# JNSresearcher/eddy_currents_3d

Measured on AMD Instinct MI355X. Metric: DOF*iters/s (fp64 BiCGSTAB-with-restart, 7-pt A-V operator), higher is better.
Workload: dtype f64

## Files before the change

eddy_currents_3d_amd/csrc/ec3d_context.hip:

```cpp
#include "../../include/ec3d_hip.h"
#include "ec3d_internal.hpp"
#include "ec3d_split_sweeps.hpp"
#include "ec3d_sweep_lists.hpp"

#include <climits>
#include <algorithm>
#include <array>
#include <cmath>
#include <cstdio>
#include <cstdlib>
#include <cstring>
#include <chrono>
#include <memory>
#include <mutex>
#include <optional>

static thread_local std::string g_err;
thread_local double *ec3d_itmax_print_hold = nullptr;
void ec3d_set_error(const std::string &msg) { g_err = msg; }
extern "C" const char *ec3d_last_error(void) { return g_err.c_str(); }

static int64_t round_up(int64_t v, int64_t m) { return (v + m - 1) / m * m; }

extern "C" void ec3d_format_real8(double v, char *buf) { ec3d_format_list_directed(v, buf); }
// ... 268 lines not shown
    static std::optional<int> env(const char *name)
    {
        const char *e = getenv(name);
        return e ? std::optional<int>(atoi(e)) : std::nullopt;
    }
    std::optional<int> nt = env("EC3D_NT"), keep = env("EC3D_KEEP");
    std::optional<int> xcd_map = env("EC3D_XCD_MAP"), vec_depth = env("EC3D_VEC_DEPTH");
    enum { K2, K4, K5, SPMV_PLAIN, NVEC };
    std::optional<int> nblk_k[NVEC] = {env("EC3D_NBLK_K2"), env("EC3D_NBLK_K4"), env("EC3D_NBLK_K5"), env("EC3D_NBLK_SPMV_PLAIN")};
    std::optional<int> map_k[NVEC] = {env("EC3D_MAP_K2"), env("EC3D_MAP_K4"), env("EC3D_MAP_K5"), env("EC3D_MAP_SPMV_PLAIN")};
    std::optional<int> depth_k[NVEC] = {env("EC3D_DEPTH_K2"), env("EC3D_DEPTH_K4"), env("EC3D_DEPTH_K5"),
                                        env("EC3D_DEPTH_SPMV_PLAIN")};
    std::optional<int> zmarch = env("EC3D_ZMARCH"), patch = env("EC3D_PATCH"), nblk_spmv = env("EC3D_NBLK_SPMV");
    std::optional<int> sav_patch = env("EC3D_SAV_PATCH"), sav_patch_px = env("EC3D_SAV_PATCH_PX"), sav_il = env("EC3D_SAV_IL");
    std::optional<int> fuse23 = env("EC3D_FUSE23"), fuse51 = env("EC3D_FUSE51"), k4s = env("EC3D_K4S");
};

static inline int64_t rows_streamed(const ec3d_ctx *c)
{
    return (c->A.sav && c->A.ulist) ? (c->A.ntiles_front + (int64_t)c->A.ulist_n) * EC3D_TILE : c->A.n_pad;
}

static int choose_sweep(ec3d_ctx *c)
{
    const SweepKnobs knob;
    Sweep &sw = c->sweep;
    sw = Sweep{};
    sw.bnd_last = -1;
    sw.ntiles = c->A.n_pad / EC3D_TILE;
    sw.n = c->A.n;
// ... 163 lines not shown
                c->fuse51_ok = fuse5 == 2 || (fuse5 == 1 && fuse_big);
            }
            if (use_patch) {
                ss.patch_npx = (int)(sdx / EC3D_PX);
                ss.patch_sdx = sdx;
                const int k4s = knob.k4s.value_or(1);
                const bool undivided = c->halo == 0 && !c->dist && c->nranks <= 1;
                const int64_t fuse_rows = !(k4s != 0 && A.ncls > 0) ? (int64_t)1 << 26 : undivided ? (int64_t)20 << 20 : (int64_t)1 << 25;
                const bool fuse_big = c->A.n_pad >= fuse_rows;
                const int fuse = knob.fuse23.value_or(1);
                c->fuse23_ok = fuse == 2 || (fuse == 1 && fuse_big);
                const int fuse5 = knob.fuse51.value_or(1);
                c->fuse51_ok = fuse5 == 2 || (fuse5 == 1 && fuse_big);
                c->k4s_ok = A.ncls > 0 && !A.sav && c->fuse23_ok && c->fuse51_ok && (k4s == 2 || (k4s == 1 && fuse_big));
                {
                    const int kinds = patch == 2 ? EC3D_PAIR_ALL : knob.patch ? 0 : big ? EC3D_PAIR_DEFAULT_BIG : 0;
                    const bool slab = c->halo > 0 || c->nranks > 1;
                    ss.pair = ec3d_patch_pairs_ok(tpp, ss.patch_npx, nplanes, ss.zm_pps, ss.nblk, slab, c->dist) ? kinds : 0;
                }
            }
        }
    }
    c->us_list.reset();
    c->us_host.clear();
    {
        const bool rp = ss.rp_px > 0;
        const std::vector<int32_t> &src = rp ? c->A.rp_ulist_host : c->A.ulist_host;
        if (rp) ss.ulist_n = (int)src.size();
        if (A.sav && ss.zm_tpp > 0 && ss.ulist_n > 0 && ss.nblk % 8 == 0 &&
            (int)src.size() == ss.ulist_n && (rp || ss.ulist == c->A.ulist)) {
            c->us_host = ec3d_xcd_local_order(src, ss.zm_tpp, ss.nblk);
            EC3D_HIP(upload_list(c->us_list, c->us_host));
            ss.ulist = c->us_list;
// ... 1064 lines not shown
```

eddy_currents_3d_amd/csrc/ec3d_form.hpp:

```cpp
#pragma once
#include "ec3d_internal.hpp"

enum { FMT_GENERIC = 0, FMT_DIA7 = 7, FMT_DICT7 = 107, FMT_SAV = 207 };
#define EC3D_SAV_STRIDE 16
#define EC3D_NSTAGE 4
#define EC3D_NSTAGE_RT 2

struct SpmvForm {
    int fmt;
    bool nt;
    bool zm;
    bool tail;
    bool patch;
    bool il;
    bool hs;
    bool pair;
};

inline SpmvForm ec3d_spmv_form(const MatView &A, const Sweep &sw)
{
    SpmvForm f{};
    f.fmt = A.sav ? FMT_SAV : A.nb == 7 && A.ncls > 0 ? FMT_DICT7 : A.nb == 7 ? FMT_DIA7 : FMT_GENERIC;
    f.nt = (sw.nt & 1) != 0;
    f.zm = sw.zm_tpp > 0 && sw.bnd_last < 0 && f.fmt != FMT_GENERIC;
    f.tail = f.fmt != FMT_SAV && A.has_tail;
    f.patch = f.zm && !f.tail && ((f.fmt == FMT_DICT7 && sw.patch_npx > 0) || (f.fmt == FMT_SAV && sw.rp_px > 0));
    f.il = f.zm && !f.patch && f.fmt == FMT_SAV && sw.il_planes > 0;
    f.hs = f.fmt == FMT_DICT7 && sw.halo_store != 0;
    return f;
}

inline bool ec3d_form_pair(const SpmvForm &f, const Sweep &sw, int kind)
{
    return f.patch && f.fmt == FMT_DICT7 && !f.hs && (sw.pair & kind) != 0;
}

inline size_t ec3d_form_lds(const MatView &A, const SpmvForm &f)
{
    const size_t sav_tbl = (size_t)A.ncls * EC3D_SAV_STRIDE * 8;
    if (f.il) return sav_tbl;
    if (f.patch && f.fmt == FMT_SAV) return sav_tbl + (size_t)(2 + EC3D_NSTAGE_RT) * EC3D_TILE * 8;
    if (f.patch) return (size_t)((f.fmt == FMT_DICT7 ? A.ncls * 7 + 1 : 0) & ~1) * 8 + (size_t)(f.pair ? 4 : 2) * EC3D_TILE * 8;
    if (f.fmt == FMT_DICT7) return (size_t)A.ncls * 7 * 8;
    if (f.fmt == FMT_SAV) return sav_tbl + (f.zm ? (size_t)EC3D_NSTAGE * EC3D_TILE * 8 : 0);
    return 0;
}
```

eddy_currents_3d_amd/csrc/ec3d_internal.hpp:

```cpp
#pragma once
#include <hip/hip_runtime.h>

#include "../../include/ec3d_hip.h"
#include "ec3d_own.hpp"

#include <algorithm>
#include <climits>
#include <cstdio>
#include <cstdint>
#include <string>
#include <vector>

#define EC3D_THREADS 256
#define EC3D_TILE 512
#define EC3D_SAV_MAXDOM 22
#define EC3D_MAXB 16
#define EC3D_CHUNK 64
#define EC3D_OUT_SLOTS 3
#ifndef EC3D_PX
#define EC3D_PX 128
#endif
#define EC3D_PY (EC3D_TILE / EC3D_PX)

struct MatView {
// ... 39 lines not shown
    const uint8_t *rp_flag;
    int nown;
    int64_t own_lo[4], own_hi[4];
    int64_t win_nt, win_blk, win_t0;
    int zm_pl0, zm_npl;
    int zm_plstep;
    int bnd_last;
    int halo_store;
    int part_off;
    const int32_t *ulist;
    int ulist_n;
    int il_planes = 0, il_nw = 0;
    const uint32_t *il_umask = nullptr;
    const int32_t *il_seg = nullptr;
    int pair = 0;
};

template <class SW>
__host__ __device__ inline int64_t ec3d_row_of(const SW &sw, int64_t tile, int t)
{
    if (sw.patch_npx <= 0) return tile * EC3D_TILE + 2 * (int64_t)t;
    const int64_t plane = tile / sw.zm_tpp, q = tile % sw.zm_tpp;
    const int64_t py = q / sw.patch_npx, px = q % sw.patch_npx;
    return plane * (int64_t)sw.zm_tpp * EC3D_TILE + (py * EC3D_PY + t / (EC3D_PX / 2)) * sw.patch_sdx + px * EC3D_PX +
           2 * (int64_t)(t % (EC3D_PX / 2));
}

template <class SW>
__host__ __device__ inline int64_t ec3d_phys_tile(const SW &sw, int64_t t)
{
// ... 470 lines not shown
```

eddy_currents_3d_amd/csrc/ec3d_kernels.hip:

```cpp
#include "ec3d_form.hpp"
#include "ec3d_recurrence.hpp"
#include "ec3d_sweep_lists.hpp"

#include <algorithm>
#include <cstdlib>
#include <type_traits>

typedef double d2 __attribute__((ext_vector_type(2)));
typedef double d2u __attribute__((ext_vector_type(2), aligned(8)));
typedef int i2 __attribute__((ext_vector_type(2)));

__device__ __forceinline__ double wave_sum(double v)
{
#pragma unroll
    for (int off = 32; off > 0; off >>= 1) v = v + __shfl_down(v, off, 64);
    return v;
}

template <bool PAIR> __device__ __forceinline__ int vw_tid()
{
    return PAIR ? (int)(threadIdx.x & (EC3D_THREADS - 1)) : (int)threadIdx.x;
}
template <bool PAIR> __device__ __forceinline__ int vw_half()
{
    if constexpr (PAIR) return __builtin_amdgcn_readfirstlane((int)(threadIdx.x / EC3D_THREADS));
    else return 0;
}
template <bool PAIR, class SW> __device__ __forceinline__ int vw_bid(const SW &sw)
{
    if constexpr (PAIR) return ec3d_patch_pair_virtual(sw.tpp, sw.patch_npx, (int)blockIdx.x, vw_half<PAIR>());
    else return (int)blockIdx.x;
}

template <int NV, bool PAIR = false>
__device__ __forceinline__ void block_sum(double (&v)[NV], double *lds)
{
    const int lane = threadIdx.x & 63, w = vw_tid<PAIR>() >> 6;
    if constexpr (PAIR) lds += vw_half<PAIR>() * (NV * 4);
#pragma unroll
    for (int k = 0; k < NV; ++k) {
        double t = wave_sum(v[k]);
        if (lane == 0) lds[k * 4 + w] = t;
    }
    __syncthreads();
#pragma unroll
    for (int k = 0; k < NV; ++k) v[k] = ((lds[k * 4 + 0] + lds[k * 4 + 1]) + lds[k * 4 + 2]) + lds[k * 4 + 3];
    __syncthreads();
}

template <int NV>
__device__ __forceinline__ void reduce_partials(const RedSrc &src, const int (&slot)[NV], double (&out)[NV],
                                                double *lds)
{
#pragma unroll
    for (int k = 0; k < NV; ++k) {
        double a = 0.0;
// ... 592 lines not shown
    }
#pragma unroll
    for (int m = 0; m < 5; ++m) {
        if (v0[m] != 0.0) s0 = s0 + v0[m] * xx[m].x;
        if (v1[m] != 0.0) s1 = s1 + v1[m] * xx[m].y;
    }
}

struct ZRegs {
    d2 xm, xc;
    d2 rim;
    d2 cr[2];
    double edge;
    unsigned short cc;
    uint32_t same;
};

__device__ __forceinline__ void stage_issue(const double *gp, double *stg, int k)
{
    __builtin_amdgcn_global_load_lds((const __attribute__((address_space(1))) void *)gp,
                                     (__attribute__((address_space(3))) void *)(stg + k * EC3D_TILE +
                                                                                (threadIdx.x >> 6) * 128),
                                     16, 0, 0);
}
__device__ __forceinline__ d2 stage_read(const double *stg, int k)
{
    return *reinterpret_cast<const d2 *>(stg + k * EC3D_TILE + 2 * threadIdx.x);
}
#define EC3D_VM_DRAIN                                                                                                  \
    do {                                                                                                               \
// ... 688 lines not shown
    }
    const d2 s = patch_sums<FMT>(c, tbl, cc, zm, ym, left, cx, right, yp, zp);
    s0 = s.x;
    s1 = s.y;
    *reinterpret_cast<d2 *>(nxt + 2 * t) = zp;
    z.xm = cx;
    z.xc = zp;
    if constexpr (RQ == PP_RIM_CARRIED) {
        if (rimrow) rimn_r = x.rpair(r + kdz + roff);
        V::to_carry(rimn_r, z.cr);
    } else {
        z.rim = x.form(rimn_r);
        z.edge = x.form(en_r);
    }
}
template <int FMT, bool NTB, bool PAIR, class V>
__device__ __forceinline__ void patch_pair(const MatDev<FMT> &A, const double *tbl, double *pbuf, int step, const V &x,
                                           int64_t r, int64_t tile, bool first, ZRegs &z, double &s0, double &s1,
                                           d2 &ctr)
{
    if constexpr (PatchReq<V>::mode == PP_BRANCHY) patch_pair_branchy<FMT, NTB, PAIR>(A, tbl, pbuf, step, x, r, tile, first, z, s0, s1, ctr);
    else patch_pair_fused<FMT, NTB, PAIR>(A, tbl, pbuf, step, x, r, tile, first, z, s0, s1, ctr);
}

template <int FMT, bool ZM, bool TAIL, bool NTB, bool PATCH, bool PAIR = false, class V, class SW>
__device__ __forceinline__ void spmv_pair(const MatDev<FMT> &A, const SW &sw, const PatchPos &pp, const double *tbl,
                                          double *stg, int &step, const V &x, int64_t r, int64_t tile, bool first,
                                          ZRegs &z, double &s0, double &s1, d2 &ctr)
{
    if constexpr (FMT == FMT_SAV && ZM && PATCH) {
// ... 441 lines not shown
        EC3D_IDLE2(s0, s1);
        acc[0] = acc[0] + q0 * q0;
        acc[0] = acc[0] + q1 * q1;
        acc[1] = acc[1] + s0 * q.x;
        acc[1] = acc[1] + s1 * q.y;
        acc[2] = acc[2] + s0 * s0;
        acc[2] = acc[2] + s1 * s1;
    });
    block_sum<3, PAIR>(acc, lds);
    {
        const int pslot_[3] = {P_SS, P_D2, P_D3};
        publish_partials<3, PAIR>(sw, part, pslot_, acc, lds);
    }
}

template <int FMT, bool NT, bool ZM, bool TAIL, bool PATCH, bool HS = false, bool PAIR = false>
__global__ __launch_bounds__(EC3D_WG_THREADS) __attribute__((amdgpu_waves_per_eu(4))) void k51_p_spmv_dot(
    MatDev<FMT> A, EC3D_SWEEP_OF(ZM) sw, RedSrc src, SolverState *st, int it, const double *__restrict__ rv,
    const double *__restrict__ p_old, const double *__restrict__ ap_old, double *__restrict__ p_new,
    double *__restrict__ ap_new, double *__restrict__ r0, double *__restrict__ part, double *hist, int64_t hist_cap)
{
    __shared__ double lds[(PAIR ? 2 : 1) * 8];
    EC3D_TBL_DECL;
    const int slot[2] = {P_RR, P_RR0N};
    PartialsEarly<2> pe;
    partials_request<2, PAIR>(src, slot, pe);
    const double bnorm = st->bnorm, tol = st->tol, alpha = st->alpha, omega = st->omega, rr0 = st->rr0[it & 1];
    TableEarly te;
    table_request<FMT>(A, te);
    {
        int si, kind;
// ... 13 lines not shown
    }
    const Ec3dBeta bs = ec3d_beta_step(alpha, omega, d[1], rr0, d[0], bnorm, tol);
    const double beta = bs.beta;
    const bool restart = bs.restart;
    if (lead) st->rr0[(it + 1) & 1] = bs.rr0_next;
    if (lead && restart) st->restarts = st->restarts + 1;
    table_store<FMT>(A, te, tbl);
    ZRegs zr;
    PatchPos pp{};
    int pstep = 0;
    double acc[1] = {0.0};
    walk_spmv<FMT, ZM, FMT != FMT_SAV, PATCH, PAIR>(A, sw, pp, [&](int64_t tile, auto fc) {
        EC3D_ROW_S;
        double s0, s1;
        d2 pc;
        spmv_pair<FMT, ZM, TAIL, NT, PATCH, PAIR>(A, sw, pp, tbl, stg, pstep, VecFusedP{rv, p_old, ap_old, beta, omega, restart}, r, tile,
                                            (bool)fc, zr, s0, s1, pc);
        d2 q = restart ? pc : load2<NT>(r0 + r);
        store2<NT>(p_new, r, nst, pc.x, pc.y);
        if (restart) store2<NT>(r0, r, nst, pc.x, pc.y);
        if constexpr (HS && FMT == FMT_DICT7 && ZM && PATCH) {
            if (sw.hs_mask) {
                const int64_t pl = tile / sw.tpp, kdz = A.off[6];
                const VecFusedP xp{rv, p_old, ap_old, beta, omega, restart};
                if ((sw.hs_mask & 1) && pl == 0) *reinterpret_cast<d2 *>(p_new + r - kdz) = xp.pair(r - kdz);
                if ((sw.hs_mask & 2) && pl == sw.hs_last) *reinterpret_cast<d2 *>(p_new + r + kdz) = xp.pair(r + kdz);
            }
        }
        store2<NT>(ap_new, r, nst, s0, s1);
        EC3D_MASK2(r, sw, s0, s1);
        EC3D_IDLE2(s0, s1);
        acc[0] = acc[0] + s0 * q.x;
        acc[0] = acc[0] + s1 * q.y;
    });
    block_sum<1, PAIR>(acc, lds);
    {
        const int pslot_[1] = {P_D1};
        publish_partials<1, PAIR>(sw, part, pslot_, acc, lds);
    }
}

template <bool NT>
__global__ __launch_bounds__(EC3D_THREADS) void k4_x_r_update(SweepV sw, RedSrc src_ss, RedSrc src, SolverState *st,
                                                              int it, const double *__restrict__ p,
                                                              const double *__restrict__ sv,
                                                              const double *__restrict__ as,
                                                              const double *__restrict__ r0, double *__restrict__ x,
                                                              double *__restrict__ rv, double *__restrict__ part,
                                                              double *hist, int64_t hist_cap)
{
// ... 446 lines not shown
    z.rp_sdy = sw.rp_sdy;
    z.rp_flag = sw.rp_flag;
    z.il_planes = sw.il_planes;
    z.il_nw = sw.il_nw;
    z.il_umask = sw.il_umask;
    z.il_seg = sw.il_seg;
    return z;
}
static constexpr bool form_possible(const SpmvForm &f)
{
    const bool table = f.fmt == FMT_DICT7 || f.fmt == FMT_SAV;
    return (!f.tail || f.fmt != FMT_SAV) && (!f.zm || f.fmt != FMT_GENERIC) && (!f.patch || (f.zm && !f.tail && table)) &&
           (!f.il || (f.zm && !f.patch && f.fmt == FMT_SAV)) && (!f.hs || f.fmt == FMT_DICT7);
}
struct SpmvFamily {
    static constexpr bool hs = false;
    static constexpr int pair_kind = EC3D_PAIR_K13;
    static constexpr bool has(const SpmvForm &f) { return form_possible(f) && !f.hs; }
};
struct FusedFamily {
    static constexpr bool hs = true;
    static constexpr bool has(const SpmvForm &f) { return form_possible(f) && f.zm && f.patch && !f.tail; }
};
struct Fused23Family : FusedFamily { static constexpr int pair_kind = EC3D_PAIR_K23; };
struct Fused51Family : FusedFamily { static constexpr int pair_kind = EC3D_PAIR_K51; };
struct K4sFamily {
    static constexpr bool hs = false;
    static constexpr int pair_kind = EC3D_PAIR_K4S;
    static constexpr bool has(const SpmvForm &f) { return FusedFamily::has(f) && f.fmt == FMT_DICT7 && !f.hs; }
};
template <int FMT_, bool NT_, bool ZM_, bool TAIL_, bool PATCH_, bool HS_, bool PAIR_> struct FormTag {
    static constexpr int FMT = FMT_;
    static constexpr bool NT = NT_, ZM = ZM_, TAIL = TAIL_, PATCH = PATCH_, HS = HS_, PAIR = PAIR_;
    static constexpr int threads = PAIR_ ? 2 * EC3D_THREADS : EC3D_THREADS;
    static int grid(const Sweep &sw) { return PAIR_ ? sw.nblk / 2 : sw.nblk; }
};
template <class FAMILY, class LAUNCH>
static void launch_form(const char *kernel, const MatView &A, const Sweep &sw, LAUNCH &&launch, int pair_kind = FAMILY::pair_kind)
{
    SpmvForm f = ec3d_spmv_form(A, sw);
    f.hs = f.hs && FAMILY::hs;
    f.pair = ec3d_form_pair(f, sw, pair_kind);
    const size_t lds = ec3d_form_lds(A, f);
    bool found = false;
    auto with_fmt = [&](auto FMT) {
        tag_bools([&](auto NT, auto ZM, auto TAIL, auto PATCH, auto IL, auto HS, auto PAIR) {
            constexpr SpmvForm cf{decltype(FMT)::value,   decltype(NT)::value, decltype(ZM)::value, decltype(TAIL)::value,
                                  decltype(PATCH)::value, decltype(IL)::value, decltype(HS)::value, decltype(PAIR)::value};
            if constexpr (FAMILY::has(cf) && (!cf.pair || (cf.patch && cf.fmt == FMT_DICT7 && !cf.hs))) {
                using T = FormTag<cf.fmt, cf.nt, cf.zm, cf.tail || cf.il, cf.patch, cf.hs, cf.pair>;
                found = true;
                if constexpr (cf.zm) launch(T{}, mat_dev<cf.fmt>(A), sweep_z(sw), lds);
                else launch(T{}, mat_dev<cf.fmt>(A), sw, lds);
            }
        }, f.nt, f.zm, f.tail, f.patch, f.il, f.hs, f.pair);
    };
    switch (f.fmt) {
    case FMT_SAV: with_fmt(std::integral_constant<int, FMT_SAV>{}); break;
    case FMT_DICT7: with_fmt(std::integral_constant<int, FMT_DICT7>{}); break;
    case FMT_DIA7: with_fmt(std::integral_constant<int, FMT_DIA7>{}); break;
    default: with_fmt(std::integral_constant<int, FMT_GENERIC>{});
    }
    if (!found) {
        char msg[160];
        snprintf(msg, sizeof msg, "%s: no kernel instance for the form fmt=%d nt=%d zm=%d tail=%d patch=%d il=%d hs=%d", kernel,
                 f.fmt, f.nt, f.zm, f.tail, f.patch, f.il, f.hs);
        ec3d_set_error(msg);
    }
}
static inline SweepV sweep_v(const Sweep &sw)
// ... 90 lines not shown
                     const double *ap, double *sv, double *as, double *part, hipStream_t s)
{
    launch_form<Fused23Family>("k23_s_spmv_dots", A, sw, [&](auto t, const auto &Ad, const auto &swk, size_t lds) {
        using T = decltype(t);
        k23_s_spmv_dots<T::FMT, T::NT, T::ZM, T::TAIL, T::PATCH, T::HS, T::PAIR><<<T::grid(sw), T::threads, lds, s>>>(
            Ad, swk, src, st, it, r, ap, sv, as, part);
    });
}

void ec3d_launch_k51(const MatView &A, const Sweep &sw, const RedSrc &src, SolverState *st, int it, const double *r,
                     const double *p_old, const double *ap_old, double *p_new, double *ap_new, double *r0, double *part,
                     double *hist, int64_t hist_cap, hipStream_t s)
{
    launch_form<Fused51Family>("k51_p_spmv_dot", A, sw, [&](auto t, const auto &Ad, const auto &swk, size_t lds) {
        using T = decltype(t);
        k51_p_spmv_dot<T::FMT, T::NT, T::ZM, T::TAIL, T::PATCH, T::HS, T::PAIR><<<T::grid(sw), T::threads, lds, s>>>(
            Ad, swk, src, st, it, r, p_old, ap_old, p_new, ap_new, r0, part, hist, hist_cap);
    });
}

void ec3d_launch_k4(const Sweep &sw, const RedSrc &src_ss, const RedSrc &src, SolverState *st, int it,
                    const double *p, const double *sv, const double *as, const double *r0, double *x, double *r,
                    double *part, double *hist, int64_t hist_cap, hipStream_t s)
{
    tag_bools([&](auto NT) {
        k4_x_r_update<decltype(NT)::value><<<sw.nblk, EC3D_THREADS, 0, s>>>(sweep_v(sw), src_ss, src, st, it, p, sv, as, r0, x, r, part,
                                                                          hist, hist_cap);
    }, nt_of(sw));
}

void ec3d_launch_k4d(const Sweep &sw, const RedSrc &src_ss, const RedSrc &src, SolverState *st, int it, int ne, int xm,
// ... 121 lines not shown
```

eddy_currents_3d_amd/csrc/ec3d_measure.hip:

```cpp
#include "../../include/ec3d_hip.h"
#include "ec3d_internal.hpp"

#include <algorithm>
#include <climits>
#include <cmath>
#include <cstdio>
#include <cstdlib>
#include <cstring>
#include <mutex>
#include <string>

extern "C" int ec3d_time_iterations(ec3d_handle c, int32_t iters, double *ms_total)
{
    int rc = ec3d_need_matrix(c, "ec3d_time_iterations");
    if (rc) return rc;
    if ((rc = ec3d_single_rank_only(c, "ec3d_time_iterations"))) return rc;
    const MatView A = c->A.view();
    c->hist_cap = 0;
    if ((rc = ec3d_launch_begin(c, A, -1.0))) return rc;
    EC3D_HIP(hipEventRecord(c->t0, c->stream));
    (void)ec3d_run_open(c, 1, iters);
    for (int it = 1; it <= iters; ++it) ec3d_launch_iteration(c, A, it);
    EC3D_HIP(hipEventRecord(c->t1, c->stream));
    EC3D_HIP(hipGetLastError());
// ... 18 lines not shown
    int rc = ec3d_need_matrix(c, "ec3d_get_fusion");
    if (rc) return rc;
    if (k2_in_k3) *k2_in_k3 = ec3d_fused23(c) ? 1 : 0;
    if (k5_in_k1) *k5_in_k1 = ec3d_fused51(c) ? 1 : 0;
    return 0;
}

extern "C" int ec3d_get_patch_rows(ec3d_handle c, int kind, int32_t *rows)
{
    int rc = ec3d_need_matrix(c, "ec3d_get_patch_rows");
    if (rc) return rc;
    if (kind < 0 || kind > 4 || !rows) return 2;
    const Sweep &ss = c->sweep_s;
    const bool dict = c->A.ncls > 0 && !c->A.sav;
    *rows = !(ss.patch_npx > 0 && dict) ? 0 : (ss.pair & (1 << kind)) ? 2 * EC3D_PY : EC3D_PY;
    return 0;
}

extern "C" int ec3d_get_x_interval(ec3d_handle c, int32_t *iterations)
{
    int rc = ec3d_need_matrix(c, "ec3d_get_x_interval");
    if (rc) return rc;
    if (iterations) *iterations = ec3d_xdefer(c);
    return 0;
}

extern "C" int ec3d_get_x_groups(ec3d_handle c, int32_t *second_stream, int32_t *groups_launched)
{
    int rc = ec3d_need_matrix(c, "ec3d_get_x_groups");
    if (rc) return rc;
// ... 115 lines not shown
```

eddy_currents_3d_amd/csrc/ec3d_sweep_lists.hpp:

```cpp
#pragma once
#include <algorithm>
#include <array>
#include <cmath>
#include <cstdint>
#include <cstdlib>
#include <vector>

inline double ec3d_pick_patch_shape(int64_t sdx, int64_t sdy, int64_t tile, int &px_out, int &py_out)
{
    double best = 0.0;
    px_out = py_out = 0;
    if (sdx % 2) return 0.0;
    for (int64_t px = 4; px <= std::min<int64_t>(sdx, 256); px += 2) {
        if (sdx % px) continue;
        if (px < 32 && px != sdx) continue;
        const int64_t py = tile / px;
        if (py < 2) continue;
        const int64_t npy = (sdy + py - 1) / py;
        const double eff = (double)(px * py) / tile * (double)sdy / (double)(npy * py);
        const bool better = eff > best + 1e-9 ||
                            (eff > best - 1e-9 && std::llabs(px - 128) < std::llabs((int64_t)px_out - 128));
        if (better) {
            best = std::max(best, eff);
            px_out = (int)px;
// ... 69 lines not shown
    if (cpx % (2 * npx)) return false;
    if (nblk % tpp) return false;
    const int64_t nseg = nblk / tpp;
    return nseg * pps == nplanes;
}
EC3D_PAIR_HD inline int ec3d_patch_pair_virtual(int tpp, int npx, int phys, int half)
{
    const int cpx = tpp >> 3, hc = cpx >> 1;
    const int c = phys & 7, sgp = phys >> 3;
    const int seg = sgp / hc, jj = sgp - seg * hc;
    const int pr = jj / npx, px = jj - pr * npx;
    return 8 * (seg * cpx + (2 * pr + half) * npx + px) + c;
}
enum { EC3D_PAIR_SPMV = 1, EC3D_PAIR_K23 = 2, EC3D_PAIR_K51 = 4, EC3D_PAIR_K4S = 8, EC3D_PAIR_K13 = 16, EC3D_PAIR_ALL = 31 };
enum { EC3D_PAIR_DEFAULT_BIG = EC3D_PAIR_SPMV | EC3D_PAIR_K23 };

inline int64_t ec3d_zm_segments(int64_t want_s, int64_t cols, int64_t max_seg, bool explicit_request)
{
    int64_t nseg = 1;
    if (explicit_request) {
        nseg = std::max<int64_t>(1, (want_s + cols / 2) / cols);
    } else {
        const int64_t fit = want_s / cols;
        nseg = (fit >= 1 && 6 * cols * fit >= 5 * want_s) ? fit : (3 * want_s + 2 * cols - 1) / (2 * cols);
    }
    return std::min<int64_t>(nseg, max_seg);
}

inline uint32_t ec3d_il_bit(const uint32_t *um, int nw, int64_t col, int64_t k)
{
// ... 103 lines not shown
```

eddy_currents_3d_amd/solver.py:

```python
from __future__ import annotations

import ctypes as C
import os

import numpy as np

PKG = os.path.dirname(os.path.abspath(__file__))
LIBPATH = os.environ.get("EC3D_LIB") or os.path.join(PKG, "libec3d_hip.so")


class EC3DError(RuntimeError):
    pass


class Geom(C.Structure):
    _fields_ = [("n_pad", C.c_int32), ("tile", C.c_int32), ("nblk", C.c_int32),
                ("threads", C.c_int32), ("xcd_group", C.c_int32), ("zm_tpp", C.c_int32),
                ("zm_pps", C.c_int32), ("ntiles_front", C.c_int32), ("ulist_n", C.c_int32),
                ("patch_x", C.c_int32), ("patch_y", C.c_int32), ("patch_sdx", C.c_int32),
                ("patch_pitch", C.c_int32), ("patch_sdy", C.c_int32)]


class MatrixInfo(C.Structure):
    _fields_ = [("n", C.c_int64), ("n_pad", C.c_int64), ("nnz", C.c_int64), ("nbands", C.c_int32),
# ... 40 lines not shown
           "ec3d_iterate_begin", "ec3d_iterate", "ec3d_get_fusion", "ec3d_get_x_interval", "ec3d_get_x_groups", "ec3d_get_k4_form", "ec3d_get_band_placement", "ec3d_get_vector_placement", "ec3d_place_vectors", "ec3d_set_format", "ec3d_set_stream",
           "ec3d_assemble_poisson_slab", "ec3d_vector_layout", "ec3d_adopt_vectors",
           "ec3d_dist_configure", "ec3d_dist_step", "ec3d_dist_set_boundary_rows", "ec3d_read_state_async", "ec3d_read_state", "ec3d_get_restart_count", "ec3d_set_zmarch", "ec3d_can_overlap",
           "ec3d_rhs_step", "ec3d_post_update", "ec3d_assemble_slab", "ec3d_vtk_fields", "ec3d_vtk_fields_begin", "ec3d_vtk_fields_wait",
           "ec3d_set_structured", "ec3d_get_row_map", "ec3d_get_ulist", "ec3d_probe_csr",
           "ec3d_device_synchronize", "ec3d_format_real8",
           "ec3d_multi_create", "ec3d_multi_destroy", "ec3d_multi_ranks", "ec3d_multi_slab", "ec3d_multi_set_format",
           "ec3d_multi_assemble_poisson", "ec3d_multi_assemble", "ec3d_multi_set_matrix_csr", "ec3d_multi_size",
           "ec3d_multi_upload", "ec3d_multi_download", "ec3d_multi_solve", "ec3d_multi_solve_resident",
           "ec3d_multi_rhs_step", "ec3d_multi_post_update", "ec3d_multi_vtk_fields", "ec3d_multi_vtk_fields_begin",
           "ec3d_multi_vtk_fields_wait", "ec3d_multi_iterate_begin",
           "ec3d_multi_iterate", "ec3d_multi_synchronize", "ec3d_true_residual", "ec3d_multi_true_residual", "ec3d_get_visit_order", "ec3d_probe_csr_multi", "ec3d_multi_spmv", "ec3d_multi_api_calls", "ec3d_multi_plan", "ec3d_multi_halo_rows", "ec3d_rccl_unique_id", "ec3d_multi_create_rank", "ec3d_format_real8_gfortran", "ec3d_multi_iterate_timed", "ec3d_multi_rccl_info",
           "ec3d_set_preconditioner", "ec3d_get_preconditioner", "ec3d_precond_apply", "ec3d_set_u_rhs",
           "ec3d_set_precond_precision", "ec3d_get_precond_precision", "ec3d_set_precond_coarsening",
           "ec3d_get_precond_coarsening", "ec3d_set_precond_grid", "ec3d_get_precond_grid",
           "ec3d_domain_integrals", "ec3d_field_energy", "ec3d_domain_linkage", "ec3d_get_class_runs", "ec3d_get_patch_rows", "ec3d_set_guess_history", "ec3d_get_guess_history"]
U_RHS = {"reference": 0, "all": 1}
PRECOND = {"none": 0, "mg": 1, "block-mg": 2}
PRECOND_E_MATRIX, PRECOND_E_COARSE = 20, 21
PRECOND_PRECISION = {"fp64": 0, "fp32": 1}
PRECOND_COARSENING = {"rediscretize": 0, "aggregate": 1}

_f64 = np.ctypeslib.ndpointer(np.float64, flags="C_CONTIGUOUS")
_i32 = np.ctypeslib.ndpointer(np.int32, flags="C_CONTIGUOUS")
_i8 = np.ctypeslib.ndpointer(np.int8, flags="C_CONTIGUOUS")
_lib = None


def torch_hip_runtime():
    import importlib.util
    try:
# ... 99 lines not shown
    L.ec3d_get_k4_form.argtypes = [hp, C.POINTER(C.c_int32)]
    L.ec3d_get_band_placement.argtypes = [hp, C.c_int32, hp, C.POINTER(C.c_int32), C.POINTER(C.c_int32)]
    L.ec3d_get_vector_placement.argtypes = [hp, C.c_int32, hp, C.POINTER(C.c_int32), C.POINTER(C.c_int32), C.POINTER(C.c_double)]
    L.ec3d_place_vectors.argtypes = [hp, C.c_int32]
    L.ec3d_set_format.argtypes = [hp, C.c_int]
    L.ec3d_set_structured.argtypes = [hp, C.c_int]
    L.ec3d_get_row_map.argtypes = [hp, _i32]
    L.ec3d_dist_set_boundary_rows.argtypes = [hp, C.c_int32, np.ctypeslib.ndpointer(np.int64, flags="C_CONTIGUOUS"),
                                              np.ctypeslib.ndpointer(np.int64, flags="C_CONTIGUOUS"),
                                              C.POINTER(C.c_int32)]
    L.ec3d_probe_csr.argtypes = [C.c_int32, _f64, _i32, _i32, C.POINTER(CsrProbe)]
    L.ec3d_probe_csr_multi.argtypes = [C.c_int32, _f64, _i32, _i32, C.c_int32, C.POINTER(C.c_int32)]
    L.ec3d_get_ulist.argtypes = [hp, _i32]
    L.ec3d_get_class_runs.argtypes = [hp, C.POINTER(C.c_int64), hp, C.c_int64]
    L.ec3d_get_patch_rows.argtypes = [hp, C.c_int, C.POINTER(C.c_int32)]
    L.ec3d_set_stream.argtypes = [hp, hp]
    L.ec3d_assemble_poisson_slab.argtypes = [hp, C.c_int32, C.c_int32, C.c_int32, C.c_int32, C.c_int32, _f64, _f64]
    L.ec3d_vector_layout.argtypes = [hp] + [C.POINTER(C.c_int64)] * 4
    L.ec3d_adopt_vectors.argtypes = [hp, hp]
    L.ec3d_dist_configure.argtypes = [hp, C.c_int32, hp, hp]
    L.ec3d_dist_step.argtypes = [hp, C.c_int32, C.c_int32, C.c_double]
    L.ec3d_read_state_async.argtypes = [hp, C.c_void_p]
    L.ec3d_read_state.argtypes = [hp, C.POINTER(C.c_int32), C.POINTER(C.c_int32), C.POINTER(C.c_double)]
    L.ec3d_get_restart_count.argtypes = [hp, C.POINTER(C.c_int32)]
    L.ec3d_get_visit_order.argtypes = [hp, C.c_int, C.POINTER(C.c_int32), C.POINTER(C.c_int64), hp, hp]
    L.ec3d_true_residual.argtypes = [hp, C.POINTER(C.c_double), C.POINTER(C.c_double)]
    L.ec3d_multi_true_residual.argtypes = [hp, C.POINTER(C.c_double), C.POINTER(C.c_double)]
    L.ec3d_multi_create.argtypes = [C.POINTER(hp), C.c_int32, hp]
    L.ec3d_multi_destroy.argtypes = [hp]
    L.ec3d_multi_ranks.argtypes = [hp]
# ... 201 lines not shown
        return off, tiles[:tot.value]

    def class_runs(self) -> np.ndarray:
        cnt = C.c_int64(0)
        _chk(self.L, self.L.ec3d_get_class_runs(self.h, C.byref(cnt), None, 0), "ec3d_get_class_runs")
        out = np.zeros(cnt.value, np.uint8)
        if cnt.value:
            _chk(self.L, self.L.ec3d_get_class_runs(self.h, C.byref(cnt), out.ctypes.data, out.size), "ec3d_get_class_runs")
        return out

    def patch_rows(self, kind: int = 0) -> int:
        rows = C.c_int32(0)
        _chk(self.L, self.L.ec3d_get_patch_rows(self.h, int(kind), C.byref(rows)), "ec3d_get_patch_rows")
        return rows.value

    def set_zmarch(self, on: bool):
        _chk(self.L, self.L.ec3d_set_zmarch(self.h, int(bool(on))), "ec3d_set_zmarch")

    def set_workgroups(self, nblk: int):
        _chk(self.L, self.L.ec3d_set_workgroups(self.h, int(nblk)), "ec3d_set_workgroups")

    def solve(self, b, x0, tolerance, itmax, hist_cap: int = 0):
        x = np.array(x0, dtype=np.float64, copy=True)
        it = C.c_int32(0)
        hist = np.full((max(hist_cap, 1), 2), np.nan)
        _chk(self.L, self.L.ec3d_solve(self.h, np.ascontiguousarray(b, np.float64), x, float(tolerance),
                                       int(itmax), C.byref(it), hist.ctypes.data if hist_cap else None,
                                       hist_cap), "ec3d_solve")
        return x, it.value, hist[:hist_cap]

# ... 525 lines not shown
```

include/ec3d_hip.h:

```cpp
#ifndef EC3D_HIP_H
#define EC3D_HIP_H
#include <stdint.h>
#ifdef __cplusplus
extern "C" {
#endif

void sprsbcgstabwr_(double *valA, int32_t *irow, int32_t *jcol, int32_t *n, double *b, double *x,
                    double *tolerance, int32_t *itmax, int32_t *iter);
void ec3d_invalidate(void);

typedef struct ec3d_ctx *ec3d_handle;

int ec3d_create(ec3d_handle *h, int device);
int ec3d_destroy(ec3d_handle h);
const char *ec3d_last_error(void);

int ec3d_set_matrix_csr(ec3d_handle h, int32_t n, const double *valA, const int32_t *irow,
                        const int32_t *jcol);

int ec3d_assemble(ec3d_handle h, int32_t sdx, int32_t sdy, int32_t sdz, const int8_t *geoPHYS,
                  const int32_t *geoPHYS_C, const double *valPHYS, int32_t nsub_glob,
                  const double *BND, const double *delta, double dt);

int ec3d_assemble_poisson(ec3d_handle h, int32_t sdx, int32_t sdy, int32_t sdz, const double *BND,
// ... 167 lines not shown
    int32_t threads;
    int32_t xcd_group;
    int32_t zm_tpp;
    int32_t zm_pps;
    int32_t ntiles_front;
    int32_t ulist_n;
    int32_t patch_x, patch_y;
    int32_t patch_sdx;
    int32_t patch_pitch;
    int32_t patch_sdy;
} ec3d_geom;
int ec3d_get_reduction_geometry(ec3d_handle h, int which, ec3d_geom *g);
int ec3d_get_ulist(ec3d_handle h, int32_t *tiles);
int ec3d_get_class_runs(ec3d_handle h, int64_t *count, uint8_t *flags, int64_t cap);
int ec3d_get_patch_rows(ec3d_handle h, int kind, int32_t *rows);
int ec3d_get_visit_order(ec3d_handle h, int which, int32_t *nwg, int64_t *total, int32_t *offsets, int32_t *tiles);
int ec3d_set_zmarch(ec3d_handle h, int on);
int ec3d_set_workgroups(ec3d_handle h, int32_t nblk);

typedef struct {
    int64_t n, n_pad, nnz;
    int32_t nbands;
    int32_t band_offset[16];
    int64_t tail_rows, tail_entries_padded;
    int64_t device_bytes;
    int32_t dict_classes;
} ec3d_matrix_info;
int ec3d_get_matrix_info(ec3d_handle h, ec3d_matrix_info *info);

int ec3d_get_band_placement(ec3d_handle h, int32_t cap, double *candidate_us, int32_t *tried, int32_t *kept);
// ... 45 lines not shown
```

Measured before the change: 50.76 billion.

## Recompute A·p_old on the fly in fused k51 kernel instead of loading it

Adds a patch_pair_apc path to the fused k51 p-update/SpMV/dot kernel. It recomputes the A·p_old product for the next plane from a second LDS-staged buffer of p_old, rather than streaming the stored ap_old vector from global memory. The path is enabled by default on large undivided dictionary-format problems, and pairing is also turned on for k51 there. A ds_bpermute-based wave reduction is added for the block sum. The trade is extra LDS use and stencil arithmetic in exchange for less global memory traffic in a bandwidth-bound fp64 kernel.

```diff
diff --git a/eddy_currents_3d_amd/csrc/ec3d_context.hip b/eddy_currents_3d_amd/csrc/ec3d_context.hip
--- a/eddy_currents_3d_amd/csrc/ec3d_context.hip
+++ b/eddy_currents_3d_amd/csrc/ec3d_context.hip
@@ -306,6 +306,7 @@
     std::optional<int> zmarch = env("EC3D_ZMARCH"), patch = env("EC3D_PATCH"), nblk_spmv = env("EC3D_NBLK_SPMV");
     std::optional<int> sav_patch = env("EC3D_SAV_PATCH"), sav_patch_px = env("EC3D_SAV_PATCH_PX"), sav_il = env("EC3D_SAV_IL");
     std::optional<int> fuse23 = env("EC3D_FUSE23"), fuse51 = env("EC3D_FUSE51"), k4s = env("EC3D_K4S");
+    std::optional<int> k51_ap = env("EC3D_K51_AP");
 };
 
 static inline int64_t rows_streamed(const ec3d_ctx *c)
@@ -499,9 +500,15 @@
                 c->fuse51_ok = fuse5 == 2 || (fuse5 == 1 && fuse_big);
                 c->k4s_ok = A.ncls > 0 && !A.sav && c->fuse23_ok && c->fuse51_ok && (k4s == 2 || (k4s == 1 && fuse_big));
                 {
-                    const int kinds = patch == 2 ? EC3D_PAIR_ALL : knob.patch ? 0 : big ? EC3D_PAIR_DEFAULT_BIG : 0;
-                    const bool slab = c->halo > 0 || c->nranks > 1;
-                    ss.pair = ec3d_patch_pairs_ok(tpp, ss.patch_npx, nplanes, ss.zm_pps, ss.nblk, slab, c->dist) ? kinds : 0;
+                    const bool inst = undivided && A.ncls > 0 && !A.sav;
+                    ss.k51_ap = inst && knob.k51_ap.value_or(big && EC3D_K51_AP_DEFAULT_BIG) != 0 ? 1 : 0;
+                }
+                const bool slab = c->halo > 0 || c->nranks > 1;
+                const bool pairs_ok = ec3d_patch_pairs_ok(tpp, ss.patch_npx, nplanes, ss.zm_pps, ss.nblk, slab, c->dist);
+                if (!knob.k51_ap && !(pairs_ok && !(knob.patch && patch != 2))) ss.k51_ap = 0;
+                {
+                    const int kinds = patch == 2 ? EC3D_PAIR_ALL : knob.patch ? 0 : !big ? 0 : EC3D_PAIR_DEFAULT_BIG | (ss.k51_ap ? EC3D_PAIR_K51 : 0);
+                    ss.pair = pairs_ok ? kinds : 0;
                 }
             }
         }
diff --git a/eddy_currents_3d_amd/csrc/ec3d_form.hpp b/eddy_currents_3d_amd/csrc/ec3d_form.hpp
--- a/eddy_currents_3d_amd/csrc/ec3d_form.hpp
+++ b/eddy_currents_3d_amd/csrc/ec3d_form.hpp
@@ -1,5 +1,6 @@
 #pragma once
 #include "ec3d_internal.hpp"
+#include "ec3d_sweep_lists.hpp"
 
 enum { FMT_GENERIC = 0, FMT_DIA7 = 7, FMT_DICT7 = 107, FMT_SAV = 207 };
 #define EC3D_SAV_STRIDE 16
@@ -15,6 +16,7 @@
     bool il;
     bool hs;
     bool pair;
+    bool apc;
 };
 
 inline SpmvForm ec3d_spmv_form(const MatView &A, const Sweep &sw)
@@ -35,12 +37,29 @@
     return f.patch && f.fmt == FMT_DICT7 && !f.hs && (sw.pair & kind) != 0;
 }
 
+inline bool ec3d_form_apc(const SpmvForm &f, const Sweep &sw)
+{
+    return f.patch && f.fmt == FMT_DICT7 && !f.hs && sw.k51_ap != 0;
+}
+
+inline SpmvForm ec3d_family_form(const MatView &A, const Sweep &sw, bool fam_hs, int pair_kind, bool fam_apc)
+{
+    SpmvForm f = ec3d_spmv_form(A, sw);
+    f.hs = f.hs && fam_hs;
+    f.pair = ec3d_form_pair(f, sw, pair_kind);
+    f.apc = fam_apc && ec3d_form_apc(f, sw);
+    return f;
+}
+inline SpmvForm ec3d_k51_form(const MatView &A, const Sweep &sw) { return ec3d_family_form(A, sw, true, EC3D_PAIR_K51, true); }
+
 inline size_t ec3d_form_lds(const MatView &A, const SpmvForm &f)
 {
     const size_t sav_tbl = (size_t)A.ncls * EC3D_SAV_STRIDE * 8;
     if (f.il) return sav_tbl;
     if (f.patch && f.fmt == FMT_SAV) return sav_tbl + (size_t)(2 + EC3D_NSTAGE_RT) * EC3D_TILE * 8;
-    if (f.patch) return (size_t)((f.fmt == FMT_DICT7 ? A.ncls * 7 + 1 : 0) & ~1) * 8 + (size_t)(f.pair ? 4 : 2) * EC3D_TILE * 8;
+    if (f.patch)
+        return (size_t)((f.fmt == FMT_DICT7 ? A.ncls * 7 + 1 : 0) & ~1) * 8 +
+               (f.apc ? (size_t)4 * ((f.pair ? 2 : 1) * EC3D_PY + 2) * EC3D_PX * 8 : (size_t)(f.pair ? 4 : 2) * EC3D_TILE * 8);
     if (f.fmt == FMT_DICT7) return (size_t)A.ncls * 7 * 8;
     if (f.fmt == FMT_SAV) return sav_tbl + (f.zm ? (size_t)EC3D_NSTAGE * EC3D_TILE * 8 : 0);
     return 0;
diff --git a/eddy_currents_3d_amd/csrc/ec3d_internal.hpp b/eddy_currents_3d_amd/csrc/ec3d_internal.hpp
--- a/eddy_currents_3d_amd/csrc/ec3d_internal.hpp
+++ b/eddy_currents_3d_amd/csrc/ec3d_internal.hpp
@@ -77,6 +77,7 @@
     const uint32_t *il_umask = nullptr;
     const int32_t *il_seg = nullptr;
     int pair = 0;
+    int k51_ap = 0;
 };
 
 template <class SW>
diff --git a/eddy_currents_3d_amd/csrc/ec3d_kernels.hip b/eddy_currents_3d_amd/csrc/ec3d_kernels.hip
--- a/eddy_currents_3d_amd/csrc/ec3d_kernels.hip
+++ b/eddy_currents_3d_amd/csrc/ec3d_kernels.hip
@@ -16,6 +16,18 @@
     for (int off = 32; off > 0; off >>= 1) v = v + __shfl_down(v, off, 64);
     return v;
 }
+__device__ __forceinline__ double wave_sum_fresh(double v)
+{
+    int lane;
+    asm volatile("v_mbcnt_lo_u32_b32 %0, -1, 0\n\tv_mbcnt_hi_u32_b32 %0, -1, %0" : "=v"(lane));
+#pragma unroll
+    for (int off = 32; off > 0; off >>= 1) {
+        const int src = (lane + off < 64 ? lane + off : lane) << 2;
+        const int lo = __builtin_amdgcn_ds_bpermute(src, __double2loint(v)), hi = __builtin_amdgcn_ds_bpermute(src, __double2hiint(v));
+        v = v + __hiloint2double(hi, lo);
+    }
+    return v;
+}
 
 template <bool PAIR> __device__ __forceinline__ int vw_tid()
 {
@@ -32,14 +44,14 @@
     else return (int)blockIdx.x;
 }
 
-template <int NV, bool PAIR = false>
+template <int NV, bool PAIR = false, bool FRESH = false>
 __device__ __forceinline__ void block_sum(double (&v)[NV], double *lds)
 {
     const int lane = threadIdx.x & 63, w = vw_tid<PAIR>() >> 6;
     if constexpr (PAIR) lds += vw_half<PAIR>() * (NV * 4);
 #pragma unroll
     for (int k = 0; k < NV; ++k) {
-        double t = wave_sum(v[k]);
+        double t = FRESH ? wave_sum_fresh(v[k]) : wave_sum(v[k]);
         if (lane == 0) lds[k * 4 + w] = t;
     }
     __syncthreads();
@@ -662,6 +674,8 @@
     double edge;
     unsigned short cc;
     uint32_t same;
+    d2 pc;
+    double pedge;
 };
 
 __device__ __forceinline__ void stage_issue(const double *gp, double *stg, int k)
@@ -1380,6 +1394,127 @@
         z.edge = x.form(en_r);
     }
 }
+template <int FMT, bool PAIR>
+__device__ __forceinline__ void patch_pair_apc(const MatDev<FMT> &A, const double *tbl, double *pbuf, int step, const VecFusedP &x,
+                                               int64_t r, int64_t tile, bool first, bool up, ZRegs &z, double &s0, double &s1,
+                                               d2 &ctr)
+{
+    static_assert(FMT == FMT_DICT7, "patch_pair_apc: the dictionary form only");
+    typedef VecFusedP V;
+    constexpr int PY = PAIR ? 2 * EC3D_PY : EC3D_PY, BUF = (PY + 2) * EC3D_PX;
+    const int t = threadIdx.x, y = t / EC3D_HX, q = t % EC3D_HX;
+    double *cur = pbuf + (step & 1) * BUF + EC3D_PX, *nxt = pbuf + ((step + 1) & 1) * BUF + EC3D_PX;
+    double *pcur = cur + 2 * BUF, *pnxt = nxt + 2 * BUF;
+    const int trim = y == 0 ? t - EC3D_HX : t + EC3D_HX;
+    const int64_t sdx = A.off[5], kdz = A.off[6], tpp = kdz / EC3D_TILE;
+    const bool calc = up && !x.restart;
+    const double *__restrict__ pup = x.p + kdz;
+    unsigned short cc, cn = 0;
+    {
+        const bool kept = !first && ((z.same >> (8 * (unsigned)((tile + tpp) & 3))) & 0xFFu) != 0;
+        uint32_t w = 0;
+        if (A.same && up) w = ((const __attribute__((address_space(4))) uint32_t *)(uintptr_t)A.same)[(tile + 2 * tpp) >> 2];
+        if (first) cc = *reinterpret_cast<const unsigned short *>(A.cls + r);
+        else cc = z.cc;
+        if (up) {
+            if (kept) cn = cc;
+            else cn = *reinterpret_cast<const unsigned short *>(A.cls + r + kdz);
+        }
+        z.same = w;
+    }
+    V::Raw2 zp_r{};
+    if (first) zp_r = x.rpair(r + kdz);
+    else zp_r.q = *reinterpret_cast<const d2u *>(x.rv + r + kdz);
+    d2 p2 = d2{0.0, 0.0};
+    if (!first && calc) p2 = *reinterpret_cast<const d2u *>(pup + r + kdz);
+    const bool edge = q == 0 || q == EC3D_HX - 1;
+    const int64_t eoff = q == 0 ? -1 : 2;
+    V::Raw1 e_r{};
+    if (edge && first) e_r = x.rat(r + eoff);
+    const bool rimrow = y == 0 || y == PY - 1;
+    const int64_t roff = y == 0 ? -sdx : sdx;
+    V::Raw2 rimc_r{};
+    if (rimrow && first) rimc_r = x.rpair(r + roff);
+    d2 zm, cx;
+    if (first) {
+        const V::Raw2 zm_r = x.rpair(r - kdz), cx_r = x.rpair(r);
+        zm = x.form(zm_r);
+        cx = x.form(cx_r);
+        *reinterpret_cast<d2 *>(cur + 2 * t) = cx;
+        const d2 rimc = x.form(rimc_r);
+        if (rimrow) *reinterpret_cast<d2 *>(cur + 2 * trim) = rimc;
+    } else {
+        cx = z.xc;
+    }
+    EC3D_PATCH_BARRIER;
+    if (!first) zm = *reinterpret_cast<const d2 *>(nxt + 2 * t);
+    const d2 ym = *reinterpret_cast<const d2 *>(cur + 2 * (t - EC3D_HX));
+    const d2 yp = *reinterpret_cast<const d2 *>(cur + 2 * (t + EC3D_HX));
+    ctr = cx;
+    double left, right;
+    {
+        const double ev = first ? x.form(e_r) : z.edge;
+        const double l = __shfl_up(cx.y, 1, 64), rr = __shfl_down(cx.x, 1, 64);
+        left = q != 0 ? l : ev;
+        right = q != EC3D_HX - 1 ? rr : ev;
+    }
+    d2 prim = d2{0.0, 0.0};
+    if (!first) {
+        const d2 pym = *reinterpret_cast<const d2 *>(pcur + 2 * (t - EC3D_HX));
+        const d2 pyp = *reinterpret_cast<const d2 *>(pcur + 2 * (t + EC3D_HX));
+        const double pl = __shfl_up(z.pc.y, 1, 64), pr = __shfl_down(z.pc.x, 1, 64);
+        const double pleft = q != 0 ? pl : z.pedge, pright = q != EC3D_HX - 1 ? pr : z.pedge;
+        const d2 pm = *reinterpret_cast<const d2 *>(pnxt + 2 * t);
+        const d2 a = patch_sums<FMT>(nullptr, tbl, cn, pm, pym, pleft, z.pc, pright, pyp, p2);
+        zp_r.pv = z.pc;
+        zp_r.a = d2{calc ? a.x : 0.0, calc ? a.y : 0.0};
+        prim = y == 0 ? pym : pyp;
+    }
+    const d2 zp = x.form(zp_r);
+    V::Raw2 rimn_r{};
+    V::Raw1 en_r{};
+    d2 prim2 = d2{0.0, 0.0};
+    double pe2 = 0.0;
+    if (first && calc) p2 = *reinterpret_cast<const d2u *>(pup + r + kdz);
+    if (rimrow) {
+        if (first) {
+            rimn_r = x.rpair(r + kdz + roff);
+        } else {
+            rimn_r.q = *reinterpret_cast<const d2u *>(x.rv + r + kdz + roff);
+            if (!x.restart) rimn_r.a = *reinterpret_cast<const d2u *>(x.ap + r + kdz + roff);
+        }
+        if (calc) prim2 = *reinterpret_cast<const d2u *>(pup + r + kdz + roff);
+    }
+    if (edge) {
+        if (first) {
+            en_r = x.rat(r + kdz + eoff);
+        } else {
+            en_r.q = x.rv[r + kdz + eoff];
+            if (!x.restart) en_r.a = x.ap[r + kdz + eoff];
+        }
+        if (calc) pe2 = pup[r + kdz + eoff];
+    }
+    if (!first) {
+        rimn_r.pv = prim;
+        en_r.pv = z.pedge;
+    }
+    const d2 s = patch_sums<FMT>(nullptr, tbl, cc, zm, ym, left, cx, right, yp, zp);
+    s0 = s.x;
+    s1 = s.y;
+    *reinterpret_cast<d2 *>(nxt + 2 * t) = zp;
+    *reinterpret_cast<d2 *>(pnxt + 2 * t) = p2;
+    if (first) *reinterpret_cast<d2 *>(pcur + 2 * t) = zp_r.pv;
+    z.xc = zp;
+    z.pc = p2;
+    z.cc = cn;
+    z.edge = x.form(en_r);
+    z.pedge = pe2;
+    const d2 rimn = x.form(rimn_r);
+    if (rimrow) {
+        *reinterpret_cast<d2 *>(nxt + 2 * trim) = rimn;
+        *reinterpret_cast<d2 *>(pnxt + 2 * trim) = prim2;
+    }
+}
 template <int FMT, bool NTB, bool PAIR, class V>
 __device__ __forceinline__ void patch_pair(const MatDev<FMT> &A, const double *tbl, double *pbuf, int step, const V &x,
                                            int64_t r, int64_t tile, bool first, ZRegs &z, double &s0, double &s1,
@@ -1851,7 +1986,7 @@
     }
 }
 
-template <int FMT, bool NT, bool ZM, bool TAIL, bool PATCH, bool HS = false, bool PAIR = false>
+template <int FMT, bool NT, bool ZM, bool TAIL, bool PATCH, bool HS = false, bool PAIR = false, bool APC = false>
 __global__ __launch_bounds__(EC3D_WG_THREADS) __attribute__((amdgpu_waves_per_eu(4))) void k51_p_spmv_dot(
     MatDev<FMT> A, EC3D_SWEEP_OF(ZM) sw, RedSrc src, SolverState *st, int it, const double *__restrict__ rv,
     const double *__restrict__ p_old, const double *__restrict__ ap_old, double *__restrict__ p_new,
@@ -1895,8 +2030,12 @@
         EC3D_ROW_S;
         double s0, s1;
         d2 pc;
-        spmv_pair<FMT, ZM, TAIL, NT, PATCH, PAIR>(A, sw, pp, tbl, stg, pstep, VecFusedP{rv, p_old, ap_old, beta, omega, restart}, r, tile,
-                                            (bool)fc, zr, s0, s1, pc);
+        if constexpr (APC)
+            patch_pair_apc<FMT, PAIR>(A, tbl, stg, pstep++, VecFusedP{rv, p_old, ap_old, beta, omega, restart}, r, tile, (bool)fc,
+                                      tile + sw.tpp < sw.ntiles, zr, s0, s1, pc);
+        else
+            spmv_pair<FMT, ZM, TAIL, NT, PATCH, PAIR>(A, sw, pp, tbl, stg, pstep, VecFusedP{rv, p_old, ap_old, beta, omega, restart}, r, tile,
+                                                (bool)fc, zr, s0, s1, pc);
         d2 q = restart ? pc : load2<NT>(r0 + r);
         store2<NT>(p_new, r, nst, pc.x, pc.y);
         if (restart) store2<NT>(r0, r, nst, pc.x, pc.y);
@@ -1914,7 +2053,7 @@
         acc[0] = acc[0] + s0 * q.x;
         acc[0] = acc[0] + s1 * q.y;
     });
-    block_sum<1, PAIR>(acc, lds);
+    block_sum<1, PAIR, APC>(acc, lds);
     {
         const int pslot_[1] = {P_D1};
         publish_partials<1, PAIR>(sw, part, pslot_, acc, lds);
@@ -2391,46 +2530,50 @@
            (!f.il || (f.zm && !f.patch && f.fmt == FMT_SAV)) && (!f.hs || f.fmt == FMT_DICT7);
 }
 struct SpmvFamily {
-    static constexpr bool hs = false;
+    static constexpr bool hs = false, apc = false;
     static constexpr int pair_kind = EC3D_PAIR_K13;
     static constexpr bool has(const SpmvForm &f) { return form_possible(f) && !f.hs; }
 };
 struct FusedFamily {
-    static constexpr bool hs = true;
+    static constexpr bool hs = true, apc = false;
     static constexpr bool has(const SpmvForm &f) { return form_possible(f) && f.zm && f.patch && !f.tail; }
 };
 struct Fused23Family : FusedFamily { static constexpr int pair_kind = EC3D_PAIR_K23; };
-struct Fused51Family : FusedFamily { static constexpr int pair_kind = EC3D_PAIR_K51; };
+struct Fused51Family : FusedFamily {
+    static constexpr int pair_kind = EC3D_PAIR_K51;
+    static constexpr bool apc = true;
+};
+static_assert(Fused51Family::hs && Fused51Family::apc && Fused51Family::pair_kind == EC3D_PAIR_K51, "ec3d_k51_form (ec3d_form.hpp)");
 struct K4sFamily {
-    static constexpr bool hs = false;
+    static constexpr bool hs = false, apc = false;
     static constexpr int pair_kind = EC3D_PAIR_K4S;
     static constexpr bool has(const SpmvForm &f) { return FusedFamily::has(f) && f.fmt == FMT_DICT7 && !f.hs; }
 };
-template <int FMT_, bool NT_, bool ZM_, bool TAIL_, bool PATCH_, bool HS_, bool PAIR_> struct FormTag {
+template <int FMT_, bool NT_, bool ZM_, bool TAIL_, bool PATCH_, bool HS_, bool PAIR_, bool APC_> struct FormTag {
     static constexpr int FMT = FMT_;
-    static constexpr bool NT = NT_, ZM = ZM_, TAIL = TAIL_, PATCH = PATCH_, HS = HS_, PAIR = PAIR_;
+    static constexpr bool NT = NT_, ZM = ZM_, TAIL = TAIL_, PATCH = PATCH_, HS = HS_, PAIR = PAIR_, APC = APC_;
     static constexpr int threads = PAIR_ ? 2 * EC3D_THREADS : EC3D_THREADS;
     static int grid(const Sweep &sw) { return PAIR_ ? sw.nblk / 2 : sw.nblk; }
 };
 template <class FAMILY, class LAUNCH>
 static void launch_form(const char *kernel, const MatView &A, const Sweep &sw, LAUNCH &&launch, int pair_kind = FAMILY::pair_kind)
 {
-    SpmvForm f = ec3d_spmv_form(A, sw);
-    f.hs = f.hs && FAMILY::hs;
-    f.pair = ec3d_form_pair(f, sw, pair_kind);
+    const SpmvForm f = ec3d_family_form(A, sw, FAMILY::hs, pair_kind, FAMILY::apc);
     const size_t lds = ec3d_form_lds(A, f);
     bool found = false;
     auto with_fmt = [&](auto FMT) {
-        tag_bools([&](auto NT, auto ZM, auto TAIL, auto PATCH, auto IL, auto HS, auto PAIR) {
-            constexpr SpmvForm cf{decltype(FMT)::value,   decltype(NT)::value, decltype(ZM)::value, decltype(TAIL)::value,
-                                  decltype(PATCH)::value, decltype(IL)::value, decltype(HS)::value, decltype(PAIR)::value};
-            if constexpr (FAMILY::has(cf) && (!cf.pair || (cf.patch && cf.fmt == FMT_DICT7 && !cf.hs))) {
-                using T = FormTag<cf.fmt, cf.nt, cf.zm, cf.tail || cf.il, cf.patch, cf.hs, cf.pair>;
+        tag_bools([&](auto NT, auto ZM, auto TAIL, auto PATCH, auto IL, auto HS, auto PAIR, auto APC) {
+            constexpr SpmvForm cf{decltype(FMT)::value,   decltype(NT)::value, decltype(ZM)::value,   decltype(TAIL)::value,
+                                  decltype(PATCH)::value, decltype(IL)::value, decltype(HS)::value,   decltype(PAIR)::value,
+                                  decltype(APC)::value};
+            constexpr bool cube2d = cf.patch && cf.fmt == FMT_DICT7 && !cf.hs;
+            if constexpr (FAMILY::has(cf) && (!cf.pair || cube2d) && (!cf.apc || (cube2d && FAMILY::apc))) {
+                using T = FormTag<cf.fmt, cf.nt, cf.zm, cf.tail || cf.il, cf.patch, cf.hs, cf.pair, cf.apc>;
                 found = true;
                 if constexpr (cf.zm) launch(T{}, mat_dev<cf.fmt>(A), sweep_z(sw), lds);
                 else launch(T{}, mat_dev<cf.fmt>(A), sw, lds);
             }
-        }, f.nt, f.zm, f.tail, f.patch, f.il, f.hs, f.pair);
+        }, f.nt, f.zm, f.tail, f.patch, f.il, f.hs, f.pair, f.apc);
     };
     switch (f.fmt) {
     case FMT_SAV: with_fmt(std::integral_constant<int, FMT_SAV>{}); break;
@@ -2551,7 +2694,7 @@
 {
     launch_form<Fused51Family>("k51_p_spmv_dot", A, sw, [&](auto t, const auto &Ad, const auto &swk, size_t lds) {
         using T = decltype(t);
-        k51_p_spmv_dot<T::FMT, T::NT, T::ZM, T::TAIL, T::PATCH, T::HS, T::PAIR><<<T::grid(sw), T::threads, lds, s>>>(
+        k51_p_spmv_dot<T::FMT, T::NT, T::ZM, T::TAIL, T::PATCH, T::HS, T::PAIR, T::APC><<<T::grid(sw), T::threads, lds, s>>>(
             Ad, swk, src, st, it, r, p_old, ap_old, p_new, ap_new, r0, part, hist, hist_cap);
     });
 }
diff --git a/eddy_currents_3d_amd/csrc/ec3d_measure.hip b/eddy_currents_3d_amd/csrc/ec3d_measure.hip
--- a/eddy_currents_3d_amd/csrc/ec3d_measure.hip
+++ b/eddy_currents_3d_amd/csrc/ec3d_measure.hip
@@ -1,5 +1,6 @@
 #include "../../include/ec3d_hip.h"
 #include "ec3d_internal.hpp"
+#include "ec3d_form.hpp"
 
 #include <algorithm>
 #include <climits>
@@ -56,6 +57,15 @@
     const Sweep &ss = c->sweep_s;
     const bool dict = c->A.ncls > 0 && !c->A.sav;
     *rows = !(ss.patch_npx > 0 && dict) ? 0 : (ss.pair & (1 << kind)) ? 2 * EC3D_PY : EC3D_PY;
+    return 0;
+}
+
+extern "C" int ec3d_get_k51_ap_form(ec3d_handle c, int32_t *computed)
+{
+    int rc = ec3d_need_matrix(c, "ec3d_get_k51_ap_form");
+    if (rc) return rc;
+    if (!computed) return 2;
+    *computed = ec3d_fused51(c) && ec3d_k51_form(c->A.view(), c->sweep_s).apc ? 1 : 0;
     return 0;
 }
 
diff --git a/eddy_currents_3d_amd/csrc/ec3d_sweep_lists.hpp b/eddy_currents_3d_amd/csrc/ec3d_sweep_lists.hpp
--- a/eddy_currents_3d_amd/csrc/ec3d_sweep_lists.hpp
+++ b/eddy_currents_3d_amd/csrc/ec3d_sweep_lists.hpp
@@ -107,6 +107,7 @@
 }
 enum { EC3D_PAIR_SPMV = 1, EC3D_PAIR_K23 = 2, EC3D_PAIR_K51 = 4, EC3D_PAIR_K4S = 8, EC3D_PAIR_K13 = 16, EC3D_PAIR_ALL = 31 };
 enum { EC3D_PAIR_DEFAULT_BIG = EC3D_PAIR_SPMV | EC3D_PAIR_K23 };
+enum { EC3D_K51_AP_DEFAULT_BIG = 1 };
 
 inline int64_t ec3d_zm_segments(int64_t want_s, int64_t cols, int64_t max_seg, bool explicit_request)
 {
diff --git a/eddy_currents_3d_amd/solver.py b/eddy_currents_3d_amd/solver.py
--- a/eddy_currents_3d_amd/solver.py
+++ b/eddy_currents_3d_amd/solver.py
@@ -78,7 +78,7 @@
            "ec3d_set_preconditioner", "ec3d_get_preconditioner", "ec3d_precond_apply", "ec3d_set_u_rhs",
            "ec3d_set_precond_precision", "ec3d_get_precond_precision", "ec3d_set_precond_coarsening",
            "ec3d_get_precond_coarsening", "ec3d_set_precond_grid", "ec3d_get_precond_grid",
-           "ec3d_domain_integrals", "ec3d_field_energy", "ec3d_domain_linkage", "ec3d_get_class_runs", "ec3d_get_patch_rows", "ec3d_set_guess_history", "ec3d_get_guess_history"]
+           "ec3d_domain_integrals", "ec3d_field_energy", "ec3d_domain_linkage", "ec3d_get_class_runs", "ec3d_get_patch_rows", "ec3d_get_k51_ap_form", "ec3d_set_guess_history", "ec3d_get_guess_history"]
 U_RHS = {"reference": 0, "all": 1}
 PRECOND = {"none": 0, "mg": 1, "block-mg": 2}
 PRECOND_E_MATRIX, PRECOND_E_COARSE = 20, 21
@@ -208,6 +208,7 @@
     L.ec3d_get_ulist.argtypes = [hp, _i32]
     L.ec3d_get_class_runs.argtypes = [hp, C.POINTER(C.c_int64), hp, C.c_int64]
     L.ec3d_get_patch_rows.argtypes = [hp, C.c_int, C.POINTER(C.c_int32)]
+    L.ec3d_get_k51_ap_form.argtypes = [hp, C.POINTER(C.c_int32)]
     L.ec3d_set_stream.argtypes = [hp, hp]
     L.ec3d_assemble_poisson_slab.argtypes = [hp, C.c_int32, C.c_int32, C.c_int32, C.c_int32, C.c_int32, _f64, _f64]
     L.ec3d_vector_layout.argtypes = [hp] + [C.POINTER(C.c_int64)] * 4
@@ -439,6 +440,11 @@
         _chk(self.L, self.L.ec3d_get_patch_rows(self.h, int(kind), C.byref(rows)), "ec3d_get_patch_rows")
         return rows.value
 
+    def k51_ap_form(self) -> int:
+        v = C.c_int32(0)
+        _chk(self.L, self.L.ec3d_get_k51_ap_form(self.h, C.byref(v)), "ec3d_get_k51_ap_form")
+        return v.value
+
     def set_zmarch(self, on: bool):
         _chk(self.L, self.L.ec3d_set_zmarch(self.h, int(bool(on))), "ec3d_set_zmarch")
 
diff --git a/include/ec3d_hip.h b/include/ec3d_hip.h
--- a/include/ec3d_hip.h
+++ b/include/ec3d_hip.h
@@ -205,6 +205,7 @@
 int ec3d_get_ulist(ec3d_handle h, int32_t *tiles);
 int ec3d_get_class_runs(ec3d_handle h, int64_t *count, uint8_t *flags, int64_t cap);
 int ec3d_get_patch_rows(ec3d_handle h, int kind, int32_t *rows);
+int ec3d_get_k51_ap_form(ec3d_handle h, int32_t *computed);
 int ec3d_get_visit_order(ec3d_handle h, int which, int32_t *nwg, int64_t *total, int32_t *offsets, int32_t *tiles);
 int ec3d_set_zmarch(ec3d_handle h, int on);
 int ec3d_set_workgroups(ec3d_handle h, int32_t nblk);
```

After: 52.41 billion, median of 6. +3.2%, better.
